# DonggeunYu/Text2Speech

Measured on AMD Instinct MI355X. Metric: WaveGlow forward audio samples/sec (batch 8x16000 per GPU), higher is better.
Workload: dtype bf16x3 (split-bf16 products, f32 accumulate); 1 GPU; WaveGlow forward, batch 8 x 16000 samples per GPU, 12 flows, n_group 8, WN 8 layers x 512 channels (reference waveglow/config.json); per_gpu_batch=8, segment_length=16000, mode=forward, parallelism=replicas, no collective

## Files before the change

text2speech_amd/csrc/conv_gemm.hip:

```cpp
#include "t2s_common.h"
#include "t2s_kernels.h"

#define B_PLANE_BYTES 16384

static __device__ __forceinline__ int swz4(int rb) {
    return (0x78 >> (rb * 2)) & 3;
}

static __device__ __forceinline__ void glds16(const void* gsrc, void* lds_dst) {
    __builtin_amdgcn_global_load_lds((const __attribute__((address_space(1))) void*)gsrc,
                                     (__attribute__((address_space(3))) void*)lds_dst, 16, 0, 0);
}

template <int EPI, int MT, bool SH = false, int NS = 2, bool X0 = false, bool RAG = false, class FMT = T2sFmt, bool A1 = false>
__global__ __launch_bounds__(512) void conv_gemm_kernel(const ConvGemmArgs a) {
    typedef typename FMT::frag8 fragT;
    constexpr int WN = 4;
    constexpr int NTH = 128 * WN;
    constexpr int NWT = 16 / WN;
    constexpr int CALL_BYTES = NTH * 16;
    constexpr int A_PLANE = MT * 64;
    constexpr int STAGE = 2 * A_PLANE + 2 * B_PLANE_BYTES;
    constexpr int MW = MT / 32;
    extern __shared__ __attribute__((aligned(16))) char smem[];
// ... 322 lines not shown
#pragma unroll
            for (int n = 0; n < NWT; ++n)
                if constexpr (!A1) acc[m][n] = FMT::mfma(al, bh[n], acc[m][n]);
#pragma unroll
            for (int n = 0; n < NWT; ++n) acc[m][n] = FMT::mfma(ah, bl[n], acc[m][n]);
#pragma unroll
            for (int n = 0; n < NWT; ++n) acc[m][n] = FMT::mfma(ah, bh[n], acc[m][n]);
            ah = ah_n;
            al = al_n;
        }
    };
    issue_a(0, 0);
    for (int u = wave; u < n_units; u += 2 * WN) issue_bunit(0, u, 0);
    asm volatile("s_waitcnt vmcnt(0)" ::: "memory");
    __syncthreads();
    const int rbase = wc * (NWT * 16) + (lane & 15);
    const int n_tap_steps = 3 * xc;
    for (int i = 0; i < n_tap_steps; ++i) {
        const int c = i / 3, tap = i - 3 * c;
        if (i + 1 < n_tap_steps) {
            const int c1 = (i + 1) / 3, tap1 = (i + 1) - 3 * c1;
            issue_a(tap1 * xc + c1, (i + 1) & 1);
        } else if (a.sc > 0) {
            issue_cond(0, (i + 1) & 1);
        }
        if (c + 1 < xc) {
            const int u = tap * (2 * WN) + wave;
            if (u < n_units) issue_bunit(c + 1, u, (c + 1) & 1);
        }
        const int row = rbase + tap * d;
        const int boff = row * 64 + (((lane >> 4) ^ swz4((row >> 2) & 3)) * 16);
        compute(Ar0 + (i & 1) * AR, Bx0 + (c & 1) * 2 * BX_PLANE, boff);
        asm volatile("s_waitcnt vmcnt(0)" ::: "memory");
        __syncthreads();
    }
    {
        const int boff0 = rbase * 64 + (((lane >> 4) ^ swz4((rbase >> 2) & 3)) * 16);
        for (int j = 0; j < a.sc; ++j) {
            const int st = (n_tap_steps + j) & 1;
            if (j + 1 < a.sc) issue_cond(j + 1, st ^ 1);
            compute(Ar0 + st * AR, Bx0 + st * 2 * BX_PLANE, boff0);
            asm volatile("s_waitcnt vmcnt(0)" ::: "memory");
            __syncthreads();
        }
    }
  }

    const int tcol = lane & 15;
    const int rq = (lane >> 4) * 4;
    if (EPI == EPI_GATE) {
        f32x4 facc[NWT];
#pragma unroll
        for (int n = 0; n < NWT; ++n) facc[n] = (f32x4){0.f, 0.f, 0.f, 0.f};
#pragma unroll
        for (int pair = 0; pair < MW / 4; ++pair) {
            u16x4 hv[2][NWT], lv[2][NWT];
#pragma unroll
            for (int half = 0; half < 2; ++half) {
                const int mp = pair * 2 + half;
                const int prow = mt * MT + wr * (MT / 2) + mp * 32 + rq;
                const f32x4 bt = *(const f32x4*)(a.bias + prow);
                const f32x4 bs = *(const f32x4*)(a.bias + prow + 16);
                const int ch = mt * (MT / 2) + wr * (MT / 4) + mp * 16 + rq;
                const bool chv = ch < a.C;
                const size_t obase = (((size_t)b * a.oc + (ch >> 5)) * a.Lp + a.halo) * 32 + (ch & 31);
#pragma unroll
                for (int n = 0; n < NWT; ++n) {
                    const int t = t0 + wc * (NWT * 16) + n * 16 + tcol;
                    u16x4 hi = {0, 0, 0, 0}, lo = {0, 0, 0, 0};
                    if (chv && t < a.L) {
                        u16x4 thi, tlo, ghi, glo;
#pragma unroll
                        for (int e = 0; e < 4; ++e) {
                            const float tv = fast_tanh(acc[2 * mp][n][e] + bt[e]);
                            const float gv = fast_sigmoid(acc[2 * mp + 1][n][e] + bs[e]);
                            u16 h, l;
                            split_fmt<FMT>(tv * gv, h, l);
                            hi[e] = h;
                            lo[e] = l;
                            split_fmt<FMT>(tv, h, l);
                            thi[e] = h;
                            tlo[e] = l;
                            split_fmt<FMT>(gv, h, l);
                            ghi[e] = h;
                            glo[e] = l;
                        }
                        const size_t o = obase + (size_t)t * 32;
                        *(u16x4*)(a.O_hi + o) = hi;
                        *(u16x4*)(a.O_lo + o) = lo;
                        if (a.T_hi) {
                            *(u16x4*)(a.T_hi + o) = thi;
                            *(u16x4*)(a.T_lo + o) = tlo;
                        }
                        if (a.G_hi) {
                            *(u16x4*)(a.G_hi + o) = ghi;
                            *(u16x4*)(a.G_lo + o) = glo;
                        }
                    }
                    hv[half][n] = hi;
                    lv[half][n] = lo;
                }
            }
            if (a.fold_A) {
                const u16* fa = a.fold_A + ((size_t)(mt * (MT / 64) + wr * (MT / 128) + pair) * 2 * 64 + lane) * 8;
                const fragT wh = *(const fragT*)fa;
                const fragT wl = *(const fragT*)(fa + 64 * 8);
#pragma unroll
                for (int n = 0; n < NWT; ++n) {
                    typedef __attribute__((ext_vector_type(8))) unsigned short u16x8;
                    const u16x8 bh8 = {hv[0][n][0], hv[0][n][1], hv[0][n][2], hv[0][n][3],
                                       hv[1][n][0], hv[1][n][1], hv[1][n][2], hv[1][n][3]};
                    const u16x8 bl8 = {lv[0][n][0], lv[0][n][1], lv[0][n][2], lv[0][n][3],
                                       lv[1][n][0], lv[1][n][1], lv[1][n][2], lv[1][n][3]};
                    const fragT bh = __builtin_bit_cast(fragT, bh8);
                    const fragT bl = __builtin_bit_cast(fragT, bl8);
                    facc[n] = FMT::mfma(wl, bh, facc[n]);
                    facc[n] = FMT::mfma(wh, bl, facc[n]);
                    facc[n] = FMT::mfma(wh, bh, facc[n]);
                }
            }
        }
        if (a.fold_A && lane < 32) {
            const int slot = mt * 2 + wr;
#pragma unroll
            for (int n = 0; n < NWT; ++n) {
                const int t = t0 + wc * (NWT * 16) + n * 16 + tcol;
                if (t >= a.L) continue;
#pragma unroll
                for (int e = 0; e < 4; ++e) {
                    float* dst = a.fold_acc + ((((size_t)slot * a.B + b) * 8 + rq + e) * a.L + t);
                    *dst = a.fold_init ? facc[n][e] : *dst + facc[n][e];
                }
            }
        }
    } else if (EPI == EPI_RESSKIP && PREX && (X0 || a.pair8)) {
      if constexpr (PREX) {
#pragma unroll
        for (int m = 0; m < MW; m += 2) {
            const int prow = mt * MT + wr * (MT / 2) + m * 16 + rq;
            const int ch = (prow & ~31) + 2 * rq;
            if (ch >= a.n_res) continue;
            const f32x4 b0 = *(const f32x4*)(a.bias + prow), b1 = *(const f32x4*)(a.bias + prow + 16);
            const size_t base = (((size_t)b * a.oc + (ch >> 5)) * a.Lp + a.halo) * 32 + (ch & 31);
#pragma unroll
            for (int n = 0; n < NWT; ++n) {
                const int t = t0 + wc * (NWT * 16) + n * 16 + tcol;
                if (t >= a.L) continue;
                u16x8_t hi, lo;
                if constexpr (RAG) {
                    if (t >= len_b) {
                        hi = lo = (u16x8_t){0, 0, 0, 0, 0, 0, 0, 0};
                        *(u16x8_t*)(a.O_hi + base + (size_t)t * 32) = hi;
                        *(u16x8_t*)(a.O_lo + base + (size_t)t * 32) = lo;
// ... 244 lines not shown
```

text2speech_amd/csrc/conv_gemm_args.h:

```cpp
#pragma once
#include "../../include/t2s_hip.h"
#include "t2s_api_common.h"
#include "t2s_kernels.h"

#include <string.h>


static inline int gate_tile_rows(int B, int C, int L) {
    const long wg256 = (long)cdiv(C, 128) * cdiv(L, 256) * B;
    return (wg256 <= 128 && C % 64 == 0) ? 128 : 256;
}
static inline int bias_act_tile_rows(int B, int Cout, int L) { return (long)cdiv(Cout, 256) * cdiv(L, 256) * B <= 64 ? 128 : 256; }
static inline int lockstep_tile_rows(int B, int C, int L) { return cdiv(C, 256) * cdiv(L, 256) * B < 200 ? 128 : 256; }
static inline int accumulate_tile_rows(int B, int Cout, int L) {
    const int wg256 = cdiv(Cout, 256) * cdiv(L, 256) * B;
    return (wg256 <= 128 || Cout % 256 == 0) && wg256 < 200 ? 128 : 256;
}
static inline bool bwd_pp256(const ConvGemmArgs& a, int rows) {
    return t2s_pp_shape_ok(a) && (long)cdiv(rows, 256) * a.n_ttiles * a.B >= 100;
}


static inline bool geometry_ok(int B, int L, int Lp, int halo, int Mpad, int rows) {
    return B > 0 && L > 0 && Lp == t2s_plane_rows(L, halo) && Mpad % 256 == 0 && Mpad >= rows;
}
static inline bool taps_ok(int taps, int dilation, int halo) {
    return taps > 0 && (taps & 1) && dilation > 0 && (taps / 2) * dilation <= halo;
}
static inline bool gate_shape_ok(int B, int C, int taps, int dilation, int L, int Lp, int halo, int Mpad) {
    return C > 0 && C % 4 == 0 && taps_ok(taps, dilation, halo) && geometry_ok(B, L, Lp, halo, Mpad, cdiv(C, 128) * 256);
}
static inline bool fold_ok(const void* fold_A, const float* fold_acc, int C) { return fold_A && fold_acc && al16(fold_A) && C % 16 == 0; }

struct ConvGemm {
    ConvGemmArgs a;

    ConvGemm(const void* A_hi, const void* A_lo, const float* bias) {
        memset(&a, 0, sizeof(a));
        a.A_hi = (const u16*)A_hi; a.A_lo = (const u16*)A_lo; a.bias = bias;
    }
    void geometry(int B, int L, int Lp, int halo, int Mpad) {
        a.B = B; a.L = L; a.Lp = Lp; a.halo = halo; a.Mpad = Mpad;
        a.n_ttiles = cdiv(L, 256);
    }
    void k_side(const void* X_hi, const void* X_lo, int xc, int taps, int dil, const void* S_hi = nullptr, const void* S_lo = nullptr,
                int sc = 0, int xbs = 0) {
        a.X_hi = (const u16*)X_hi; a.X_lo = (const u16*)X_lo; a.xc = xc; a.xbs = xbs;
        a.S_hi = (const u16*)S_hi; a.S_lo = (const u16*)S_lo; a.sc = sc;
        a.taps = taps; a.dil = dil;
        a.nk_x = taps * xc; a.nk = a.nk_x + sc;
    }
    void output(void* O_hi, void* O_lo, int oc) { a.O_hi = (u16*)O_hi; a.O_lo = (u16*)O_lo; a.oc = oc; }
    void fold(const void* fold_A, float* fold_acc, int fold_init) {
        a.fold_A = (const u16*)fold_A; a.fold_acc = fold_acc; a.fold_init = fold_init;
    }
    hipError_t launch(int epi, int rows, int mt_rows, void* stream, bool bwd_pp = false, bool h16 = false) {
        a.n_mtiles = cdiv(rows, mt_rows);
        if (h16) return t2s_launch_conv_gemm(a, epi, (hipStream_t)stream, mt_rows, true);
        if (a.ph_P > 0) return t2s_launch_gate_gemm_pp(a, (hipStream_t)stream);
        if (bwd_pp) return t2s_launch_bwd_gemm_pp(a, epi, (hipStream_t)stream);
        return t2s_launch_conv_gemm(a, epi, (hipStream_t)stream, mt_rows);
    }
};
```

text2speech_amd/csrc/gate_gemm_pp.hip:

```cpp
#include "t2s_common.h"
#include "t2s_kernels.h"

#include <stdlib.h>

#include <type_traits>

namespace {

constexpr int PP_PLANE = 16384;
constexpr int PP_HALF = 8192;
constexpr int PP_BUF = 4 * PP_PLANE;

__device__ __forceinline__ void pp_store8(u16* dst, u16x4 v) { *(u16x4*)dst = v; }

__device__ __forceinline__ int pp_swz4(int rb) { return (0x78 >> (rb * 2)) & 3; }

__device__ __forceinline__ void pp_glds16(const void* gsrc, void* lds_dst) {
    __builtin_amdgcn_global_load_lds((const __attribute__((address_space(1))) void*)gsrc,
                                     (__attribute__((address_space(3))) void*)lds_dst, 16, 0, 0);
}

struct BCursor {
    long off;
    long aoff;
// ... 276 lines not shown
    PP_STAMP(1)
    for (; ks + 2 < nk; ++ks) kstep(ks, std::true_type{});
    for (; ks < nk; ++ks) kstep(ks, std::false_type{});
    if (wr == 0) __builtin_amdgcn_s_barrier();
    PP_STAMP(2)
#undef PP_MFMA

    const int tcol = lane & 15;
    const int rq = (lane >> 4) * 4;
    int cb[4], ct[4];
    bool cok[4];
#pragma unroll
    for (int n = 0; n < 4; ++n) {
        const int col = (n >> 1) * 128 + wc * 32 + (n & 1) * 16 + tcol;
        if constexpr (PH) {
            const int bl = col / a.ph_FT, fl = col - bl * a.ph_FT;
            cb[n] = b + bl;
            ct[n] = a.ph_P * (ft * a.ph_FT + fl) + phi;
        } else {
            cb[n] = b;
            ct[n] = t0 + col;
        }
        cok[n] = cb[n] < a.B && ct[n] < a.L;
    }
  if constexpr (EPI == EPI_GATE) {
    f32x4 bt_all[4], bs_all[4];
#pragma unroll
    for (int mp = 0; mp < 4; ++mp) {
        const int prow = mt * 256 + (mp >> 1) * 128 + wr * 64 + (mp & 1) * 32 + rq;
        bt_all[mp] = *(const f32x4*)(a.bias + prow);
        bs_all[mp] = *(const f32x4*)(a.bias + prow + 16);
    }
    fragT fw_h[2] = {}, fw_l[2] = {};
    if (a.fold_A) {
#pragma unroll
        for (int pair = 0; pair < 2; ++pair) {
            const u16* fa = a.fold_A + ((size_t)(mt * 4 + pair * 2 + wr) * 2 * 64 + lane) * 8;
            fw_h[pair] = *(const fragT*)fa;
            fw_l[pair] = *(const fragT*)(fa + 64 * 8);
        }
    }
    f32x4 facc[4];
#pragma unroll
    for (int n = 0; n < 4; ++n) facc[n] = (f32x4){0.f, 0.f, 0.f, 0.f};
    if (a.fold_A && !a.fold_init && lane < 32) {
        const int slot = mt * 2 + wr;
#pragma unroll
        for (int n = 0; n < 4; ++n) {
            const int tc = cok[n] ? ct[n] : 0, bc = cok[n] ? cb[n] : 0;
#pragma unroll
            for (int e = 0; e < 4; ++e) facc[n][e] = a.fold_acc[(((size_t)slot * a.B + bc) * 8 + rq + e) * a.L + tc];
        }
    }
#pragma unroll
    for (int pair = 0; pair < 2; ++pair) {
        u16x4 hv[2][4], lv[2][4];
#pragma unroll
        for (int half = 0; half < 2; ++half) {
            const int mp = pair * 2 + half;
            constexpr float L2E = 1.4426950408889634f;
            const f32x4 bt = bt_all[mp] * (2.0f * L2E), bs = bs_all[mp] * (-L2E);
            const int ch = mt * 128 + pair * 64 + wr * 32 + half * 16 + rq;
            const bool chv = ch < a.C;
            const size_t obase = ((size_t)(ch >> 5) * a.Lp + a.halo) * 32 + (ch & 31);
#pragma unroll
            for (int n = 0; n < 4; ++n) {
                u16x4 hi = {0, 0, 0, 0}, lo = {0, 0, 0, 0};
                if (chv && cok[n]) {
                    const size_t o = obase + ((size_t)cb[n] * a.oc * a.Lp + (size_t)ct[n]) * 32;
                    if (a.G_hi) {
                        u16x4 thi, tlo, ghi, glo;
#pragma unroll
                        for (int e = 0; e < 4; ++e) {
                            const float E = __builtin_amdgcn_exp2f(fminf(fmaf(acc[2 * mp][n][e], 2.0f * L2E, bt[e]), 20.0f * L2E));
                            const float F = __builtin_amdgcn_exp2f(fmaf(acc[2 * mp + 1][n][e], -L2E, bs[e]));
                            const float tv = (E - 1.0f) * __builtin_amdgcn_rcpf(E + 1.0f);
                            const float gv = __builtin_amdgcn_rcpf(1.0f + F);
                            u16 h, l;
                            split_fmt<FMT>(tv * gv, h, l);
                            hi[e] = h;
                            lo[e] = l;
                            split_fmt<FMT>(tv, h, l);
                            thi[e] = h;
                            tlo[e] = l;
                            split_fmt<FMT>(gv, h, l);
                            ghi[e] = h;
                            glo[e] = l;
                        }
                        if (a.T_hi) {
                            pp_store8(a.T_hi + o, thi);
                            pp_store8(a.T_lo + o, tlo);
                        }
                        pp_store8(a.G_hi + o, ghi);
                        pp_store8(a.G_lo + o, glo);
                    } else {
#pragma unroll
                        for (int e = 0; e < 4; ++e) {
                            const float E = __builtin_amdgcn_exp2f(fminf(fmaf(acc[2 * mp][n][e], 2.0f * L2E, bt[e]), 20.0f * L2E));
                            const float F = __builtin_amdgcn_exp2f(fmaf(acc[2 * mp + 1][n][e], -L2E, bs[e]));
                            const float v = (E - 1.0f) * __builtin_amdgcn_rcpf((E + 1.0f) * (1.0f + F));
                            u16 h, l;
                            split_fmt<FMT>(v, h, l);
                            hi[e] = h;
                            lo[e] = l;
                        }
                    }
                    pp_store8(a.O_hi + o, hi);
                    pp_store8(a.O_lo + o, lo);
                }
                hv[half][n] = hi;
                lv[half][n] = lo;
            }
        }
        if (a.fold_A) {
            const fragT wh = fw_h[pair], wl = fw_l[pair];
#pragma unroll
            for (int n = 0; n < 4; ++n) {
                typedef __attribute__((ext_vector_type(8))) unsigned short u16x8;
                const u16x8 bh8 = {hv[0][n][0], hv[0][n][1], hv[0][n][2], hv[0][n][3],
                                   hv[1][n][0], hv[1][n][1], hv[1][n][2], hv[1][n][3]};
                const u16x8 bl8 = {lv[0][n][0], lv[0][n][1], lv[0][n][2], lv[0][n][3],
                                   lv[1][n][0], lv[1][n][1], lv[1][n][2], lv[1][n][3]};
                const fragT bh = __builtin_bit_cast(fragT, bh8);
                const fragT bl = __builtin_bit_cast(fragT, bl8);
                facc[n] = FMT::mfma(wl, bh, facc[n]);
                facc[n] = FMT::mfma(wh, bl, facc[n]);
                facc[n] = FMT::mfma(wh, bh, facc[n]);
            }
        }
    }
    if (a.fold_A && lane < 32) {
        const int slot = mt * 2 + wr;
#pragma unroll
        for (int n = 0; n < 4; ++n) {
            if (!cok[n]) continue;
#pragma unroll
            for (int e = 0; e < 4; ++e) {
                a.fold_acc[(((size_t)slot * a.B + cb[n]) * 8 + rq + e) * a.L + ct[n]] = facc[n][e];
            }
        }
    }
  } else if constexpr (EPI == EPI_RESSKIP) {
    typedef __attribute__((ext_vector_type(8))) unsigned short u16x8_t;
    if (a.pair8) {
#pragma unroll
      for (int m0 = 0; m0 < 8; m0 += 2) {
        const int grp = mt * 256 + (m0 >> 2) * 128 + wr * 64 + (m0 & 3) * 16;
        const bool rok = grp < a.n_res;
        const int chc = rok ? grp + 2 * rq : 0;
        const f32x4 b0 = *(const f32x4*)(a.bias + chc), b1 = *(const f32x4*)(a.bias + chc + 4);
        const size_t ob = ((size_t)(chc >> 5) * a.Lp + a.halo) * 32 + (chc & 31);
        u16x8_t oh[4], ol[4];
#pragma unroll
        for (int n = 0; n < 4; ++n) {
            oh[n] = (u16x8_t){0, 0, 0, 0, 0, 0, 0, 0};
            ol[n] = oh[n];
            if (rok && cok[n] && !a.res_init) {
                const size_t o = ob + ((size_t)cb[n] * a.oc * a.Lp + (size_t)ct[n]) * 32;
                oh[n] = *(const u16x8_t*)((a.R_hi ? a.R_hi : a.O_hi) + o);
                ol[n] = *(const u16x8_t*)((a.R_lo ? a.R_lo : a.O_lo) + o);
            }
        }
        if (!rok) continue;
#pragma unroll
// ... 207 lines not shown
```

text2speech_amd/csrc/t2s_api.hip:

```cpp
#include "../../include/t2s_hip.h"
#include "t2s_kernels.h"
#include "t2s_api_common.h"
#include "conv_gemm_args.h"

#include <stdlib.h>
#include <string.h>

static thread_local char g_hip_err[256] = "";

extern "C" int t2s_internal_fail_hip(int ei) {
    hipError_t e = (hipError_t)ei;
    strncpy(g_hip_err, hipGetErrorString(e), sizeof(g_hip_err) - 1);
    g_hip_err[sizeof(g_hip_err) - 1] = 0;
    return T2S_EHIP;
}


static inline bool a_operand_ok(const void* A_hi, const void* A_lo, bool h16) { return h16 ? (A_hi && al16(A_hi)) : planes_ok(A_hi, A_lo); }

static int pack_table(const t2s_pack_job* jobs, int n_jobs, long total_rows, void* stream, bool h16) {
    if (!jobs || n_jobs <= 0 || total_rows <= 0 || total_rows > 0x7fffffffL) return T2S_EINVAL;
    static_assert(sizeof(t2s_pack_job) == sizeof(PackJob), "t2s_pack_job layout");
    T2S_CHECK_HIP(t2s_launch_pack_table((const PackJob*)jobs, n_jobs, total_rows, (hipStream_t)stream, h16));
    return T2S_OK;
}

static int upsample_squeeze(const float* mel, const float* W, const float* bias, int B, int n_mel, int frames, int ksize, int stride,
                            int n_group, int L, int Lp, int halo, void* S_hi, void* S_lo, void* stream, bool h16) {
    if (!mel || !W || !bias || !S_hi || !S_lo) return T2S_EINVAL;
    if (B <= 0 || n_mel <= 0 || frames <= 0 || L <= 0 || n_group <= 0 || stride <= 0 || ksize % stride) return T2S_EINVAL;
    if (!al16(W) || !al16(S_hi) || !al16(S_lo)) return T2S_EINVAL;
    if (Lp < t2s_plane_rows(L, halo)) return T2S_EINVAL;
    if ((long)L * n_group > (long)(frames - 1) * stride + ksize) return T2S_EINVAL;
    if (n_group == 8 && (stride % 8 || ksize % 8)) return T2S_EINVAL;
    T2S_CHECK_HIP(t2s_launch_upsample_squeeze(mel, W, bias, B, n_mel, frames, ksize, stride, n_group, L, Lp, halo,
                                              (u16*)S_hi, (u16*)S_lo, (hipStream_t)stream, h16));
    return T2S_OK;
}

static int wg_start(const float* z, const float* w, const float* bias, int B, int n_group, int c_off, int n_half, int C, int L, int Lp,
                    int halo, void* X_hi, void* X_lo, void* stream, bool h16, const int* lengths = nullptr) {
    if (!z || !w || !bias || !X_hi || !X_lo) return T2S_EINVAL;
    if (B <= 0 || L <= 0 || C <= 0 || n_half <= 0 || n_half > 8 || c_off < 0 || c_off + n_half > n_group) return T2S_EINVAL;
    if (!al16(X_hi) || !al16(X_lo) || Lp < t2s_plane_rows(L, halo)) return T2S_EINVAL;
    T2S_CHECK_HIP(t2s_launch_start(z, w, bias, B, n_group, c_off, n_half, C, L, Lp, halo, (u16*)X_hi, (u16*)X_lo,
                                   (hipStream_t)stream, 0, 0, nullptr, nullptr, lengths, h16));
    return T2S_OK;
}

static int endfold_weights(const t2s_endfold_job* jobs, int n_jobs, int C, void* stream, bool h16) {
    if (!jobs || n_jobs <= 0 || C <= 0 || (size_t)8 * C * sizeof(float) > 60 * 1024) return T2S_EINVAL;
    static_assert(sizeof(t2s_endfold_job) == sizeof(EndFoldJob), "t2s_endfold_job layout");
    T2S_CHECK_HIP(t2s_launch_endfold_weights((const EndFoldJob*)jobs, n_jobs, C, (hipStream_t)stream, h16));
    return T2S_OK;
}

static int in_cond_gate_fold(const void* A_hi, const void* A_lo, const float* bias, const void* X_hi, const void* X_lo,
                             const void* S_hi, const void* S_lo, void* acts_hi, void* acts_lo, const void* fold_A, float* fold_acc,
                             int fold_init, int B, int C, int n_cond, int taps, int dilation, int L, int Lp, int halo, int Mpad,
                             void* stream, bool h16, const int* lengths = nullptr) {
    if (!a_operand_ok(A_hi, A_lo, h16) || !planes_ok(X_hi, X_lo) || !planes_ok(acts_hi, acts_lo) || !bias || !al16(bias)) return T2S_EINVAL;
    if ((n_cond > 0 && !planes_ok(S_hi, S_lo)) || !fold_ok(fold_A, fold_acc, C)) return T2S_EINVAL;
    if (!gate_shape_ok(B, C, taps, dilation, L, Lp, halo, Mpad)) return T2S_EINVAL;
    ConvGemm g(A_hi, A_lo, bias);
    g.geometry(B, L, Lp, halo, Mpad);
    g.k_side(X_hi, X_lo, cdiv(C, 32), taps, dilation, S_hi, S_lo, cdiv(n_cond, 32));
    g.output(acts_hi, acts_lo, cdiv(C, 32));
    g.fold(fold_A, fold_acc, fold_init);
    g.a.C = C;
    g.a.lengths = lengths;
    T2S_CHECK_HIP(g.launch(EPI_GATE, 2 * C, gate_tile_rows(B, C, L), stream, false, h16));
    return T2S_OK;
}

extern "C" {

int t2s_abi_version(void) { return 4; }

int t2s_sizeof_taco_decoder(void) { return (int)sizeof(t2s_taco_decoder); }
int t2s_sizeof_taco_bptt(void) { return (int)sizeof(t2s_taco_bptt); }

int t2s_operand_format(void) {
#ifdef T2S_SPLIT_F16
    return 1;
#else
    return 0;
#endif
}

const char* t2s_error_string(int code) {
    switch (code) {
        case T2S_OK: return "ok";
        case T2S_EINVAL: return "invalid argument";
        case T2S_EHIP: return "HIP runtime error";
        default: return "unknown error";
    }
}
const char* t2s_last_hip_error(void) { return g_hip_err; }

int t2s_plane_rows(int L, int halo) { return cdiv(L, 256) * 256 + 2 * halo; }
int t2s_padded_rows(int rows) { return cdiv(rows, 256) * 256; }

int t2s_pack_conv_weight(const float* v, const float* g, int g_is_scale, const float* bias_in, int O, int Cin, int Kt,
                         int perm, int C_gate, int row_off, int Mpad, int koff, int Cin_pad, void* A_hi, void* A_lo,
                         float* bias_out, int bias_accumulate, void* stream) {
    if (!v || !A_hi || !A_lo || O <= 0 || Cin <= 0 || Kt <= 0) return T2S_EINVAL;
    if (Mpad % 256 || koff % 32 || Cin_pad % 32 || Cin_pad < Cin) return T2S_EINVAL;
    if (perm == T2S_PERM_GATE) {
        if (O != 2 * C_gate || cdiv(C_gate, 128) * 256 > Mpad) return T2S_EINVAL;
    } else if (perm == T2S_PERM_NONE) {
        if (row_off < 0 || row_off + O > Mpad) return T2S_EINVAL;
    } else {
        return T2S_EINVAL;
    }
// ... 153 lines not shown
    ConvGemm g(A_hi, A_lo, bias);
    g.geometry(B, L, Lp, halo, Mpad);
    g.k_side(acts_hi, acts_lo, cdiv(C, 32), 1, 1);
    g.output(X_hi, X_lo, cdiv(C, 32));
    g.a.skip = skip; g.a.C = C; g.a.n_res = n_res; g.a.skip_init = skip_init;
    T2S_CHECK_HIP(g.launch(EPI_RESSKIP, n_res + C, 256, stream));
    return T2S_OK;
}

int t2s_wg_endfold_weights(const t2s_endfold_job* jobs, int n_jobs, int C, void* stream) {
    return endfold_weights(jobs, n_jobs, C, stream, false);
}
int t2s_wg_endfold_weights_h16(const t2s_endfold_job* jobs, int n_jobs, int C, void* stream) {
    return endfold_weights(jobs, n_jobs, C, stream, true);
}

int t2s_wg_gate_tile_rows(int B, int C, int L) {
    if (B <= 0 || C <= 0 || L <= 0) return T2S_EINVAL;
    return gate_tile_rows(B, C, L);
}

int t2s_wg_gate_fold_slots(int B, int C, int L) {
    if (B <= 0 || C <= 0 || L <= 0) return T2S_EINVAL;
    return gate_tile_rows(B, C, L) == 128 ? 2 * cdiv(C, 64) : 2 * cdiv(C, 128);
}

int t2s_wg_in_cond_gate_fold(const void* A_hi, const void* A_lo, const float* bias, const void* X_hi, const void* X_lo,
                             const void* S_hi, const void* S_lo, void* acts_hi, void* acts_lo, const void* fold_A,
                             float* fold_acc, int fold_init, int B, int C, int n_cond, int taps, int dilation, int L,
                             int Lp, int halo, int Mpad, void* stream) {
    return in_cond_gate_fold(A_hi, A_lo, bias, X_hi, X_lo, S_hi, S_lo, acts_hi, acts_lo, fold_A, fold_acc, fold_init, B, C, n_cond, taps,
                             dilation, L, Lp, halo, Mpad, stream, false);
}
int t2s_wg_in_cond_gate_fold_h16(const void* A_hi, const void* A_lo, const float* bias, const void* X_hi, const void* X_lo,
                                 const void* S_hi, const void* S_lo, void* acts_hi, void* acts_lo, const void* fold_A,
                                 float* fold_acc, int fold_init, int B, int C, int n_cond, int taps, int dilation, int L,
                                 int Lp, int halo, int Mpad, void* stream) {
    return in_cond_gate_fold(A_hi, A_lo, bias, X_hi, X_lo, S_hi, S_lo, acts_hi, acts_lo, fold_A, fold_acc, fold_init, B, C, n_cond, taps,
                             dilation, L, Lp, halo, Mpad, stream, true);
}
int t2s_wg_in_cond_gate_fold_h16_ragged(const void* A_hi, const void* A_lo, const float* bias, const void* X_hi, const void* X_lo,
                                        const void* S_hi, const void* S_lo, void* acts_hi, void* acts_lo, const void* fold_A,
                                        float* fold_acc, int fold_init, int B, int C, int n_cond, int taps, int dilation, int L,
                                        int Lp, int halo, int Mpad, const int* lengths, void* stream) {
    if (!lengths) return T2S_EINVAL;
    return in_cond_gate_fold(A_hi, A_lo, bias, X_hi, X_lo, S_hi, S_lo, acts_hi, acts_lo, fold_A, fold_acc, fold_init, B, C, n_cond, taps,
                             dilation, L, Lp, halo, Mpad, stream, true, lengths);
}

int t2s_wg_in_win_gate_fold(const void* A_hi, const void* A_lo, const float* bias, const void* W_hi, const void* W_lo,
                            const void* S_hi, const void* S_lo, void* acts_hi, void* acts_lo, const void* fold_A,
                            float* fold_acc, int fold_init, int B, int C, int n_cond, int win_chunks, int L, int Lp, int halo,
                            int Mpad, void* stream) {
    if (!planes_ok(A_hi, A_lo) || !planes_ok(W_hi, W_lo) || !planes_ok(S_hi, S_lo) || !planes_ok(acts_hi, acts_lo) || !bias ||
        !al16(bias))
        return T2S_EINVAL;
    if (!fold_ok(fold_A, fold_acc, C) || C <= 0 || n_cond <= 0 || halo < 0 || (win_chunks != 2 && win_chunks != 4)) return T2S_EINVAL;
    if (!geometry_ok(B, L, Lp, halo, Mpad, cdiv(C, 128) * 256)) return T2S_EINVAL;
    ConvGemm g(A_hi, A_lo, bias);
    g.geometry(B, L, Lp, halo, Mpad);
    g.k_side(W_hi, W_lo, win_chunks, 1, 1, S_hi, S_lo, cdiv(n_cond, 32));
    g.output(acts_hi, acts_lo, cdiv(C, 32));
    g.fold(fold_A, fold_acc, fold_init);
    g.a.C = C;
    T2S_CHECK_HIP(g.launch(EPI_GATE, 2 * C, gate_tile_rows(B, C, L), stream));
    return T2S_OK;
}

int t2s_wg_upsample_basis(const float* W, const float* bias, int n_mel, int ksize, int stride, int n_group, int Lp, int halo,
                          void* U_hi, void* U_lo, void* stream) {
    if (!W || !bias || !planes_ok(U_hi, U_lo)) return T2S_EINVAL;
    if (n_mel <= 0 || n_group <= 0 || stride <= 0 || ksize <= 0 || ksize % stride || stride % n_group) return T2S_EINVAL;
    const int ncols = (stride / n_group) * (ksize / stride) * n_mel + 1;
    if (halo < 0 || Lp != t2s_plane_rows(ncols, halo)) return T2S_EINVAL;
    T2S_CHECK_HIP(t2s_launch_upbasis_planes(W, bias, n_mel, ksize, stride, n_group, Lp, halo, (u16*)U_hi, (u16*)U_lo,
                                            (hipStream_t)stream));
    return T2S_OK;
}

int t2s_wg_compose_cond(const float* tmp, const float* bias_in, int rows, int Mpad, int P, int K2, long ld, void* A2_hi,
                        void* A2_lo, float* bias_out, void* stream) {
    if (!tmp || !bias_in || !bias_out || !planes_ok(A2_hi, A2_lo)) return T2S_EINVAL;
    if (rows <= 0 || Mpad % 256 || rows > Mpad || P <= 0 || K2 <= 0 || K2 % 32 || ld < (long)P * K2 + 1) return T2S_EINVAL;
    T2S_CHECK_HIP(t2s_launch_compose_pack(tmp, bias_in, rows, Mpad, P, K2, (int)ld, (u16*)A2_hi, (u16*)A2_lo, bias_out,
                                          (hipStream_t)stream));
    return T2S_OK;
}

int t2s_wg_melwin_planes(const float* mel, int B, int n_mel, int frames, int nlag, int Fp, void* M_hi, void* M_lo, void* stream) {
    if (!mel || !planes_ok(M_hi, M_lo)) return T2S_EINVAL;
    if (B <= 0 || n_mel <= 0 || frames <= 0 || nlag <= 0 || Fp < frames) return T2S_EINVAL;
    T2S_CHECK_HIP(t2s_launch_melwin_planes(mel, B, n_mel, frames, nlag, Fp, (u16*)M_hi, (u16*)M_lo, (hipStream_t)stream));
    return T2S_OK;
}

int t2s_wg_in_melwin_gate_fold(const void* A_hi, const void* A_lo, const void* A2_hi, const void* A2_lo, const float* bias,
                               const void* X_hi, const void* X_lo, const void* M_hi, const void* M_lo, void* acts_hi,
                               void* acts_lo, const void* fold_A, float* fold_acc, int fold_init, int B, int C, int K2,
                               int taps, int dilation, int L, int Lp, int halo, int Mpad, int P, int Fp, void* stream) {
    if (!planes_ok(A_hi, A_lo) || !planes_ok(A2_hi, A2_lo) || !planes_ok(X_hi, X_lo) || !planes_ok(M_hi, M_lo) ||
        !planes_ok(acts_hi, acts_lo) || !bias || !al16(bias))
        return T2S_EINVAL;
    if (!fold_ok(fold_A, fold_acc, C) || !gate_shape_ok(B, C, taps, dilation, L, Lp, halo, Mpad)) return T2S_EINVAL;
    if (K2 <= 0 || K2 % 32 || P <= 0) return T2S_EINVAL;
    const int F = cdiv(L, P);
    if (Fp < F || gate_tile_rows(B, C, L) != 256) return T2S_EINVAL;
    ConvGemm g(A_hi, A_lo, bias);
    g.geometry(B, L, Lp, halo, Mpad);
    g.k_side(X_hi, X_lo, cdiv(C, 32), taps, dilation, M_hi, M_lo, K2 / 32);
    g.output(acts_hi, acts_lo, cdiv(C, 32));
    g.fold(fold_A, fold_acc, fold_init);
    g.a.A2_hi = (const u16*)A2_hi; g.a.A2_lo = (const u16*)A2_lo;
    g.a.C = C;
    g.a.n_ttiles = 0;
    g.a.ph_P = P; g.a.ph_Fp = Fp;
    g.a.ph_FT = F <= 64 ? 64 : (F <= 128 ? 128 : 256);
    g.a.ph_bper = 256 / g.a.ph_FT;
    g.a.ph_nft = cdiv(F, g.a.ph_FT);
    T2S_CHECK_HIP(g.launch(EPI_GATE, 2 * C, 256, stream));
    return T2S_OK;
}

static int res_only(const void* A_hi, const void* A_lo, const float* bias, const void* acts_hi, const void* acts_lo,
                    void* X_hi, void* X_lo, int B, int C, int L, int Lp, int halo, int Mpad, int pair8, const int* lengths,
                    void* stream, bool h16 = false) {
    if (!a_operand_ok(A_hi, A_lo, h16) || !planes_ok(acts_hi, acts_lo) || !planes_ok(X_hi, X_lo) || !bias || !al16(bias)) return T2S_EINVAL;
    if (C <= 0 || C % 4 || (pair8 && C % 32) || !geometry_ok(B, L, Lp, halo, Mpad, C)) return T2S_EINVAL;
    ConvGemm g(A_hi, A_lo, bias);
    g.geometry(B, L, Lp, halo, Mpad);
    g.k_side(acts_hi, acts_lo, cdiv(C, 32), 1, 1);
    g.output(X_hi, X_lo, cdiv(C, 32));
    g.a.C = 0; g.a.n_res = C; g.a.pair8 = pair8 ? 1 : 0;
    g.a.lengths = lengths;
    T2S_CHECK_HIP(g.launch(EPI_RESSKIP, C, 128, stream, false, h16));
    return T2S_OK;
}

int t2s_wg_res_only_h16(const void* A_hi, const void* A_lo, const float* bias, const void* acts_hi, const void* acts_lo,
                        void* X_hi, void* X_lo, int B, int C, int L, int Lp, int halo, int Mpad, int pair8, void* stream) {
    return res_only(A_hi, A_lo, bias, acts_hi, acts_lo, X_hi, X_lo, B, C, L, Lp, halo, Mpad, pair8, nullptr, stream, true);
}

int t2s_wg_res_only(const void* A_hi, const void* A_lo, const float* bias, const void* acts_hi, const void* acts_lo,
                    void* X_hi, void* X_lo, int B, int C, int L, int Lp, int halo, int Mpad, int pair8, void* stream) {
    return res_only(A_hi, A_lo, bias, acts_hi, acts_lo, X_hi, X_lo, B, C, L, Lp, halo, Mpad, pair8, nullptr, stream);
}

int t2s_wg_res_only_ragged(const void* A_hi, const void* A_lo, const float* bias, const void* acts_hi, const void* acts_lo,
                           void* X_hi, void* X_lo, int B, int C, int L, int Lp, int halo, int Mpad, int pair8, const int* lengths,
                           void* stream) {
    if (!lengths) return T2S_EINVAL;
    return res_only(A_hi, A_lo, bias, acts_hi, acts_lo, X_hi, X_lo, B, C, L, Lp, halo, Mpad, pair8, lengths, stream);
}

// ... 121 lines not shown
```

text2speech_amd/csrc/t2s_kernels.h:

```cpp
#pragma once
#include <hip/hip_runtime.h>
#include <stdint.h>

typedef unsigned short u16;

enum { EPI_GATE = 0, EPI_RESSKIP = 1, EPI_BIAS_ACT = 2, EPI_GATE_BWD = 3 };
enum { ACT_NONE = 0, ACT_RELU = 1, ACT_TANH = 2 };
enum { PERM_NONE = 0, PERM_GATE = 1, PERM_PAIR8 = 2 };

struct ConvGemmArgs {
    const u16* A_hi;
    const u16* A_lo;
    const u16* X_hi;
    const u16* X_lo;
    const u16* S_hi;
    const u16* S_lo;
    const float* bias;
    u16* O_hi;
    u16* O_lo;
    float* skip;
    float* out_f32;
    int nk;
    int nk_x;
    int xc, sc, oc;
    int xbs;
    int taps, dil;
    int Mpad, Lp, halo, L, B;
    int n_mtiles, n_ttiles;
    int C;
    int n_res;
    int skip_init;
    int act;
    int f32_cl;
    u16* T_hi;
    u16* T_lo;
    u16* G_hi;
    u16* G_lo;
    int tc;
    int pair8;
    int res_init;
    const u16* R_hi;
    const u16* R_lo;
    long a_bstride;
    int ksplit;
    int k0, kchunk, kend;
    int kflat;
    const u16* fold_A;
    float* fold_acc;
    int fold_init;
    const u16* A2_hi;
    const u16* A2_lo;
    int ph_P;
    int ph_FT;
    int ph_bper;
    int ph_nft;
    int ph_Fp;
    const float* x0_z;
    const float* x0_w;
    const float* x0_b;
    int x0_G, x0_coff, x0_nh;
    const int* lengths;
};

#define T2S_RAG_SKIP_COLS 256
#ifdef __HIPCC__
static __device__ __forceinline__ void t2s_rag_zero_fold(const ConvGemmArgs& a, int mt, int b, int t0, int tid) {
    if (!a.fold_A || !a.fold_init) return;
    const int ncols = min(T2S_RAG_SKIP_COLS, a.L - t0);
    for (int idx = tid; idx < 16 * T2S_RAG_SKIP_COLS; idx += 512) {
        const int col = idx % T2S_RAG_SKIP_COLS, sj = idx / T2S_RAG_SKIP_COLS;
        if (col < ncols) a.fold_acc[(((size_t)(mt * 2 + (sj >> 3)) * a.B + b) * 8 + (sj & 7)) * a.L + t0 + col] = 0.f;
    }
}
#endif

hipError_t t2s_launch_conv_gemm(const ConvGemmArgs& a, int epi, hipStream_t stream, int mt_rows = 256, bool h16 = false);
hipError_t t2s_launch_gate_gemm_pp(const ConvGemmArgs& a, hipStream_t stream, bool h16 = false);
hipError_t t2s_launch_bwd_gemm_pp(const ConvGemmArgs& a, int epi, hipStream_t stream);
bool t2s_pp_shape_ok(const ConvGemmArgs& a);

struct WgradChunk {
    const u16* hi;
    const u16* lo;
    long bstride;
};
struct WgradClArgs {
    const WgradChunk* a_chunks;
    const WgradChunk* b_chunks;
    float* P;
    int M, N, ldp, n_mtiles, n_ntiles;
    int B, k0, k1;
    int nslab, kchunk;
    int bias_cols;
};
hipError_t t2s_launch_wgrad_cl(const WgradClArgs& a, hipStream_t stream);

struct PackArgs {
    const float* v;
    const float* g;
    const float* bias_in;
    u16* A_hi;
    u16* A_lo;
    float* bias_out;
    int O, Cin, Kt;
    int perm, C_gate;
    int Mpad;
    int koff;
    int Cin_pad;
    int bias_accumulate;
    int row_off;
    int g_is_scale;
};
hipError_t t2s_launch_pack(const PackArgs& a, hipStream_t stream);
struct PackJob {
    const float* v; const float* g; const float* bias_in; const float* bias_in2;
    u16* A_hi; u16* A_lo; float* bias_out;
    long row_start;
    long O, Cin, Kt, perm, C_gate, Mpad, koff, Cin_pad, row_off, g_is_scale;
    float* scale_out;
};
hipError_t t2s_launch_pack_table(const PackJob* jobs, int n_jobs, long total_rows, hipStream_t stream, bool h16 = false);
hipError_t t2s_launch_weightnorm_small(const float* v, const float* g, int O, int K, float* w, hipStream_t stream);

hipError_t t2s_launch_upbasis_planes(const float* W, const float* bias, int n_mel, int ksize, int stride, int n_group, int Lp,
                                     int halo, u16* U_hi, u16* U_lo, hipStream_t stream);
hipError_t t2s_launch_compose_pack(const float* tmp, const float* bias_in, int rows, int Mpad, int P, int K2, int ld, u16* A2_hi,
// ... 57 lines not shown
```

text2speech_amd/glow.py:

```python
import ctypes
import os
from collections import namedtuple

import torch
import torch.nn.functional as F

from . import _lib, sampling


class _WaveGlowLossFn(torch.autograd.Function):

    @staticmethod
    def forward(ctx, sigma, n_flows, z, *rest):
        log_s = [t.detach().to(torch.float32).contiguous() for t in rest[:n_flows]]
        dets = [t.detach() for t in rest[n_flows:]]
        d0 = dets[0]
        if all(t.dtype == torch.float32 and t.dim() == 0 and t.untyped_storage().data_ptr() == d0.untyped_storage().data_ptr()
               and t.storage_offset() == d0.storage_offset() + k for k, t in enumerate(dets)):
            log_det = d0.as_strided((n_flows,), (1,))
        else:
            log_det = torch.stack([t.to(torch.float32).reshape(()) for t in dets])
        zc = z.detach().to(torch.float32).contiguous()
        dev = zc.device
        d_z = torch.empty_like(zc) if z.requires_grad else None
# ... 507 lines not shown
        _lib.call(name, _lib.ptr(mel32), _lib.ptr(W), _lib.ptr(bias), B, up.in_channels,
                  mel32.size(2), up.kernel_size[0], up.stride[0], m.n_group, L, w["Lp"], g["halo"],
                  _lib.ptr(w["Sh"]), _lib.ptr(w["Sl"]), _lib.current_stream())
        self._keep += [mel32, W, bias]

    def _boundary(self, plan, k, z_in, z_out, B, L, w, prev=None, W=None):
        m, g = self.m, self.geom()
        c_off, n_rem, n_half = self._flow_geom(k)
        fold_acc = bes = b_end = log_s = None
        nslots = c_off_p = nh_p = 0
        if prev is not None:
            kp, log_s = prev
            c_off_p, _, nh_p = self._flow_geom(kp)
            fold_acc, nslots = w["fold_acc"], w["fold_acc"].size(0)
            bes = plan.pk["flows"][kp]["bes"]
            b_end = _f32c(m.WN[kp].end.bias)
            self._keep.append(b_end)
        name, lengths = plan.entry["boundary"]
        _lib.call(name, _lib.ptr(z_in), _lib.ptr(z_out), _lib.ptr(fold_acc), nslots, _lib.ptr(bes), g["nl"],
                  _lib.ptr(b_end), _lib.ptr(log_s), c_off_p, nh_p, _lib.ptr(W), c_off, n_rem, n_half, B, m.n_group, L, w["Lp"],
                  g["halo"], g["ks"], g["nwc"], _lib.ptr(w["Wh"]), _lib.ptr(w["Wl"]), *lengths, _lib.current_stream())

    def _wn(self, plan, k, z, B, L, w, c_off, n_half):
        m, g = self.m, self.geom()
        C, nl, ks = g["C"], g["nl"], g["ks"]
        path, P = plan.path, _lib.ptr
        fl = plan.pk["flows"][k]
        st = _lib.current_stream()
        b_start = _f32c(m.WN[k].start.bias)
        self._keep.append(b_start)
        X, S, win, acts = ((P(w[n + "h"]), P(w[n + "l"])) for n in "XSWA")
        if not path.boundary:
            name, lengths = plan.entry["start_window" if path.start_fold else "start"]
            window = ()
            if name in _START_TAKES_WINDOW:
                window = (ks, g["nwc"], *win) if path.start_fold else (0, 0, None, None)
            _lib.call(name, P(z), P(fl["w_start"]), P(b_start), B, m.n_group, c_off, n_half, C, L, w["Lp"], g["halo"], *X,
                      *window, *lengths, st)
        gate, gate_lengths = plan.entry["gate" if plan.melwin is None else "gate_melwin"]
        gate_window = plan.entry["gate_window"][0]
        res, res_lengths = plan.entry["res"]
        res_start, res_start_lengths = plan.entry["res_start"]
        pair8 = 1 if plan.pk["res_pair8"] else 0
        dims1 = (L, w["Lp"], g["halo"], g["Mpad1"])
        for i in range(nl):
            ly = fl["layers"][i]
            full_k = not (path.start_fold and i == 0)
            timed = full_k and self.gemm_events is not None and self._gemm_launch_no % self.gemm_event_stride == 0
            if full_k:
                self._gemm_launch_no += 1
            if timed:
                e0, e1 = torch.cuda.Event(enable_timing=True), torch.cuda.Event(enable_timing=True)
                e0.record()
            out = (*acts, P(ly["fold_A"]), P(w["fold_acc"]))
            if not full_k:
                _lib.call(gate_window, P(fl["A0h"]), P(fl["A0l"]), P(ly["b1"]), *win, *S, *out, 1, B, C, g["n_cond"], g["nwc"], *dims1, st)
            elif plan.melwin is not None:
                Mh, Ml, Fp, n_phase, K2 = plan.melwin
                _lib.call(gate, P(ly["A1h"]), P(ly["A1l"]), P(ly["Ach"]), P(ly["Acl"]), P(ly["b1c"]), *X, P(Mh), P(Ml), *out,
                          1 if i == 0 else 0, B, C, K2, ks, 2 ** i, *dims1, n_phase, Fp, st)
            else:
                _lib.call(gate, P(ly["A1h"]), P(ly["A1l"]), P(ly["b1"]), *X, *S, *out,
                          1 if i == 0 else 0, B, C, g["n_cond"], ks, 2 ** i, *dims1, *gate_lengths, st)
            if timed:
                e1.record()
                self.gemm_events.append((e0, e1))
            if i == nl - 1:
                continue
            weights = (P(ly["A2h"]), P(ly["A2l"]), P(ly["b2"]), *acts)
            dims2 = (B, C, L, w["Lp"], g["halo"], ly["Mpad2"])
            if path.boundary and i == 0:
                _lib.call(res_start, *weights, P(z), P(fl["w_start"]), P(b_start), m.n_group, c_off, n_half, *X, *dims2,
                          *res_start_lengths, st)
            else:
                _lib.call(res, *weights, *X, *dims2, pair8, *res_lengths, st)

    def wn_forward(self, k, audio, spect):
        self._check_inputs(audio, spect)
        dev = audio.device
        self._enter(dev)
        B, n_in, L = audio.shape
        c_off, n_rem, n_half = self._flow_geom(k)
        g = self.geom()
        if n_in != n_half or spect.size(1) != g["n_cond"] or spect.size(2) != L:
            raise ValueError("WN[%d] takes audio [B, %d, L] and spect [B, %d, L]" % (k, n_half, g["n_cond"]))
        plan = self._plan()
        self._keep = []
        plan = self._pack(plan, dev)
        w = self.workspace(B, L, dev)
        st = _lib.current_stream()
        spect32 = _f32c(spect)
        _lib.call("t2s_f32_to_planes", _lib.ptr(spect32), B, g["n_cond"], L, w["Lp"], g["halo"], _lib.ptr(w["Sh"]), _lib.ptr(w["Sl"]), st)
        z = torch.zeros(B, self.m.n_group, L, dtype=torch.float32, device=dev)
        z[:, c_off:c_off + n_half] = audio.detach().to(torch.float32)
        if plan.path.boundary:
            self._boundary(plan, k, z, None, B, L, w)
        self._wn(plan, k, z, B, L, w, c_off, n_half)
        wn_out =torch.empty(B, 2 * n_half, L, dtype=torch.float32, device=dev)
        self._end_fold(k, z, None, w["fold_acc"], wn_out, B, L, c_off, n_half, reverse=False, plan=plan)
        self._keep += [spect32, z]
        return wn_out.to(audio.dtype)

    def _end_fold(self, k, z, log_s, fold_acc, wn_out, B, L, c_off, n_half, reverse, plan=None):
        b_end = _f32c(self.m.WN[k].end.bias)
        self._keep.append(b_end)
        pk = self.packed if plan is None else plan.pk
        _lib.call("t2s_wg_end_fold_affine", _lib.ptr(fold_acc), fold_acc.size(0), _lib.ptr(pk["flows"][k]["bes"]),
# ... 412 lines not shown
```

Before: 8.166 million audio samples/s.

## Widen gate epilogue stores via permlane16 swap and skip dead last-layer acts

The gate GEMM epilogue now pairs the two 16-channel halves of each lane and shuffles them with permlane16_swap, so every lane issues one 16-byte store per plane where it previously issued two 8-byte stores, whenever C is a multiple of 16. Separately, the last WN layer of each flow no longer writes its gated activations, since only the folded skip/end path consumes them. The API validation now accepts null activation planes. The aim is less store traffic and fewer store instructions, at the cost of extra cross-lane permute instructions and more live registers in the epilogue.

Measured after the change: 8.211 million audio samples/s, median of 6. About the same (+0.5%).

```diff
diff --git a/text2speech_amd/csrc/conv_gemm.hip b/text2speech_amd/csrc/conv_gemm.hip
--- a/text2speech_amd/csrc/conv_gemm.hip
+++ b/text2speech_amd/csrc/conv_gemm.hip
@@ -398,53 +398,93 @@
         f32x4 facc[NWT];
 #pragma unroll
         for (int n = 0; n < NWT; ++n) facc[n] = (f32x4){0.f, 0.f, 0.f, 0.f};
+        const bool st_acts = a.O_hi != nullptr;
+        const bool st16 = (a.C & 15) == 0;
+        const int pc = t2s_gate_piece16_ch(lane);
 #pragma unroll
         for (int pair = 0; pair < MW / 4; ++pair) {
             u16x4 hv[2][NWT], lv[2][NWT];
+            f32x4 bt2[2], bs2[2];
 #pragma unroll
             for (int half = 0; half < 2; ++half) {
-                const int mp = pair * 2 + half;
-                const int prow = mt * MT + wr * (MT / 2) + mp * 32 + rq;
-                const f32x4 bt = *(const f32x4*)(a.bias + prow);
-                const f32x4 bs = *(const f32x4*)(a.bias + prow + 16);
-                const int ch = mt * (MT / 2) + wr * (MT / 4) + mp * 16 + rq;
-                const bool chv = ch < a.C;
-                const size_t obase = (((size_t)b * a.oc + (ch >> 5)) * a.Lp + a.halo) * 32 + (ch & 31);
-#pragma unroll
-                for (int n = 0; n < NWT; ++n) {
-                    const int t = t0 + wc * (NWT * 16) + n * 16 + tcol;
-                    u16x4 hi = {0, 0, 0, 0}, lo = {0, 0, 0, 0};
+                const int prow = mt * MT + wr * (MT / 2) + (pair * 2 + half) * 32 + rq;
+                bt2[half] = *(const f32x4*)(a.bias + prow);
+                bs2[half] = *(const f32x4*)(a.bias + prow + 16);
+            }
+            const int ch0 = mt * (MT / 2) + wr * (MT / 4) + pair * 32;
+            const size_t cbase = (((size_t)b * a.oc + (ch0 >> 5)) * a.Lp + a.halo) * 32;
+            const bool pv = ch0 + pc < a.C;
+#pragma unroll
+            for (int n = 0; n < NWT; ++n) {
+                const int t = t0 + wc * (NWT * 16) + n * 16 + tcol;
+                const size_t ocol = cbase + (size_t)t * 32;
+                u16x4 hi[2], lo[2], thi[2], tlo[2], ghi[2], glo[2];
+#pragma unroll
+                for (int half = 0; half < 2; ++half) {
+                    const int mp = pair * 2 + half;
+                    const f32x4 bt = bt2[half], bs = bs2[half];
+                    const int ch = ch0 + half * 16 + rq;
+                    const bool chv = ch < a.C;
+                    hi[half] = lo[half] = thi[half] = tlo[half] = ghi[half] = glo[half] = (u16x4){0, 0, 0, 0};
                     if (chv && t < a.L) {
-                        u16x4 thi, tlo, ghi, glo;
 #pragma unroll
                         for (int e = 0; e < 4; ++e) {
                             const float tv = fast_tanh(acc[2 * mp][n][e] + bt[e]);
                             const float gv = fast_sigmoid(acc[2 * mp + 1][n][e] + bs[e]);
                             u16 h, l;
                             split_fmt<FMT>(tv * gv, h, l);
-                            hi[e] = h;
-                            lo[e] = l;
+                            hi[half][e] = h;
+                            lo[half][e] = l;
                             split_fmt<FMT>(tv, h, l);
-                            thi[e] = h;
-                            tlo[e] = l;
+                            thi[half][e] = h;
+                            tlo[half][e] = l;
                             split_fmt<FMT>(gv, h, l);
-                            ghi[e] = h;
-                            glo[e] = l;
+                            ghi[half][e] = h;
+                            glo[half][e] = l;
                         }
-                        const size_t o = obase + (size_t)t * 32;
-                        *(u16x4*)(a.O_hi + o) = hi;
-                        *(u16x4*)(a.O_lo + o) = lo;
-                        if (a.T_hi) {
-                            *(u16x4*)(a.T_hi + o) = thi;
-                            *(u16x4*)(a.T_lo + o) = tlo;
+                        if (!st16) {
+                            const size_t o = ocol + (half * 16 + rq);
+                            if (st_acts) {
+                                *(u16x4*)(a.O_hi + o) = hi[half];
+                                *(u16x4*)(a.O_lo + o) = lo[half];
+                            }
+                            if (a.T_hi) {
+                                *(u16x4*)(a.T_hi + o) = thi[half];
+                                *(u16x4*)(a.T_lo + o) = tlo[half];
+                            }
+                            if (a.G_hi) {
+                                *(u16x4*)(a.G_hi + o) = ghi[half];
+                                *(u16x4*)(a.G_lo + o) = glo[half];
+                            }
                         }
-                        if (a.G_hi) {
-                            *(u16x4*)(a.G_hi + o) = ghi;
-                            *(u16x4*)(a.G_lo + o) = glo;
+                    }
+                    hv[half][n] = hi[half];
+                    lv[half][n] = lo[half];
+                }
+                if (st16) {
+                    const bool ok = pv && t < a.L;
+                    const size_t o = ocol + pc;
+                    if (st_acts) {
+                        const t2s_u32x4 h16 = t2s_gate_piece16(hi[0], hi[1]), l16 = t2s_gate_piece16(lo[0], lo[1]);
+                        if (ok) {
+                            t2s_store16(a.O_hi + o, h16);
+                            t2s_store16(a.O_lo + o, l16);
                         }
                     }
-                    hv[half][n] = hi;
-                    lv[half][n] = lo;
+                    if (a.T_hi) {
+                        const t2s_u32x4 th16 = t2s_gate_piece16(thi[0], thi[1]), tl16 = t2s_gate_piece16(tlo[0], tlo[1]);
+                        if (ok) {
+                            t2s_store16(a.T_hi + o, th16);
+                            t2s_store16(a.T_lo + o, tl16);
+                        }
+                    }
+                    if (a.G_hi) {
+                        const t2s_u32x4 gh16 = t2s_gate_piece16(ghi[0], ghi[1]), gl16 = t2s_gate_piece16(glo[0], glo[1]);
+                        if (ok) {
+                            t2s_store16(a.G_hi + o, gh16);
+                            t2s_store16(a.G_lo + o, gl16);
+                        }
+                    }
                 }
             }
             if (a.fold_A) {
diff --git a/text2speech_amd/csrc/conv_gemm_args.h b/text2speech_amd/csrc/conv_gemm_args.h
--- a/text2speech_amd/csrc/conv_gemm_args.h
+++ b/text2speech_amd/csrc/conv_gemm_args.h
@@ -30,6 +30,7 @@
 static inline bool gate_shape_ok(int B, int C, int taps, int dilation, int L, int Lp, int halo, int Mpad) {
     return C > 0 && C % 4 == 0 && taps_ok(taps, dilation, halo) && geometry_ok(B, L, Lp, halo, Mpad, cdiv(C, 128) * 256);
 }
+static inline bool acts_ok(const void* acts_hi, const void* acts_lo) { return (!acts_hi && !acts_lo) || planes_ok(acts_hi, acts_lo); }
 static inline bool fold_ok(const void* fold_A, const float* fold_acc, int C) { return fold_A && fold_acc && al16(fold_A) && C % 16 == 0; }
 
 struct ConvGemm {
diff --git a/text2speech_amd/csrc/gate_gemm_pp.hip b/text2speech_amd/csrc/gate_gemm_pp.hip
--- a/text2speech_amd/csrc/gate_gemm_pp.hip
+++ b/text2speech_amd/csrc/gate_gemm_pp.hip
@@ -352,24 +352,29 @@
             for (int e = 0; e < 4; ++e) facc[n][e] = a.fold_acc[(((size_t)slot * a.B + bc) * 8 + rq + e) * a.L + tc];
         }
     }
+    const bool st_acts = a.O_hi != nullptr;
+    const bool st16 = (a.C & 15) == 0;
+    const int pc = t2s_gate_piece16_ch(lane);
 #pragma unroll
     for (int pair = 0; pair < 2; ++pair) {
         u16x4 hv[2][4], lv[2][4];
-#pragma unroll
-        for (int half = 0; half < 2; ++half) {
-            const int mp = pair * 2 + half;
-            constexpr float L2E = 1.4426950408889634f;
-            const f32x4 bt = bt_all[mp] * (2.0f * L2E), bs = bs_all[mp] * (-L2E);
-            const int ch = mt * 128 + pair * 64 + wr * 32 + half * 16 + rq;
-            const bool chv = ch < a.C;
-            const size_t obase = ((size_t)(ch >> 5) * a.Lp + a.halo) * 32 + (ch & 31);
-#pragma unroll
-            for (int n = 0; n < 4; ++n) {
-                u16x4 hi = {0, 0, 0, 0}, lo = {0, 0, 0, 0};
+        constexpr float L2E = 1.4426950408889634f;
+        const int ch0 = mt * 128 + pair * 64 + wr * 32;
+        const size_t cbase = ((size_t)(ch0 >> 5) * a.Lp + a.halo) * 32;
+        const bool pv = ch0 + pc < a.C;
+#pragma unroll
+        for (int n = 0; n < 4; ++n) {
+            u16x4 hi[2], lo[2], thi[2], tlo[2], ghi[2], glo[2];
+            const size_t ocol = cbase + ((size_t)cb[n] * a.oc * a.Lp + (size_t)ct[n]) * 32;
+#pragma unroll
+            for (int half = 0; half < 2; ++half) {
+                const int mp = pair * 2 + half;
+                const f32x4 bt = bt_all[mp] * (2.0f * L2E), bs = bs_all[mp] * (-L2E);
+                const int ch = ch0 + half * 16 + rq;
+                const bool chv = ch < a.C;
+                hi[half] = lo[half] = thi[half] = tlo[half] = ghi[half] = glo[half] = (u16x4){0, 0, 0, 0};
                 if (chv && cok[n]) {
-                    const size_t o = obase + ((size_t)cb[n] * a.oc * a.Lp + (size_t)ct[n]) * 32;
                     if (a.G_hi) {
-                        u16x4 thi, tlo, ghi, glo;
 #pragma unroll
                         for (int e = 0; e < 4; ++e) {
                             const float E = __builtin_amdgcn_exp2f(fminf(fmaf(acc[2 * mp][n][e], 2.0f * L2E, bt[e]), 20.0f * L2E));
@@ -378,21 +383,15 @@
                             const float gv = __builtin_amdgcn_rcpf(1.0f + F);
                             u16 h, l;
                             split_fmt<FMT>(tv * gv, h, l);
-                            hi[e] = h;
-                            lo[e] = l;
+                            hi[half][e] = h;
+                            lo[half][e] = l;
                             split_fmt<FMT>(tv, h, l);
-                            thi[e] = h;
-                            tlo[e] = l;
+                            thi[half][e] = h;
+                            tlo[half][e] = l;
                             split_fmt<FMT>(gv, h, l);
-                            ghi[e] = h;
-                            glo[e] = l;
+                            ghi[half][e] = h;
+                            glo[half][e] = l;
                         }
-                        if (a.T_hi) {
-                            pp_store8(a.T_hi + o, thi);
-                            pp_store8(a.T_lo + o, tlo);
-                        }
-                        pp_store8(a.G_hi + o, ghi);
-                        pp_store8(a.G_lo + o, glo);
                     } else {
 #pragma unroll
                         for (int e = 0; e < 4; ++e) {
@@ -401,15 +400,53 @@
                             const float v = (E - 1.0f) * __builtin_amdgcn_rcpf((E + 1.0f) * (1.0f + F));
                             u16 h, l;
                             split_fmt<FMT>(v, h, l);
-                            hi[e] = h;
-                            lo[e] = l;
+                            hi[half][e] = h;
+                            lo[half][e] = l;
                         }
                     }
-                    pp_store8(a.O_hi + o, hi);
-                    pp_store8(a.O_lo + o, lo);
+                    if (!st16) {
+                        const size_t o = ocol + (half * 16 + rq);
+                        if (a.G_hi) {
+                            if (a.T_hi) {
+                                pp_store8(a.T_hi + o, thi[half]);
+                                pp_store8(a.T_lo + o, tlo[half]);
+                            }
+                            pp_store8(a.G_hi + o, ghi[half]);
+                            pp_store8(a.G_lo + o, glo[half]);
+                        }
+                        if (st_acts) {
+                            pp_store8(a.O_hi + o, hi[half]);
+                            pp_store8(a.O_lo + o, lo[half]);
+                        }
+                    }
                 }
-                hv[half][n] = hi;
-                lv[half][n] = lo;
+                hv[half][n] = hi[half];
+                lv[half][n] = lo[half];
+            }
+            if (st16) {
+                const bool ok = pv && cok[n];
+                const size_t o = ocol + pc;
+                if (a.G_hi) {
+                    if (a.T_hi) {
+                        const t2s_u32x4 th16 = t2s_gate_piece16(thi[0], thi[1]), tl16 = t2s_gate_piece16(tlo[0], tlo[1]);
+                        if (ok) {
+                            t2s_store16(a.T_hi + o, th16);
+                            t2s_store16(a.T_lo + o, tl16);
+                        }
+                    }
+                    const t2s_u32x4 gh16 = t2s_gate_piece16(ghi[0], ghi[1]), gl16 = t2s_gate_piece16(glo[0], glo[1]);
+                    if (ok) {
+                        t2s_store16(a.G_hi + o, gh16);
+                        t2s_store16(a.G_lo + o, gl16);
+                    }
+                }
+                if (st_acts) {
+                    const t2s_u32x4 h16 = t2s_gate_piece16(hi[0], hi[1]), l16 = t2s_gate_piece16(lo[0], lo[1]);
+                    if (ok) {
+                        t2s_store16(a.O_hi + o, h16);
+                        t2s_store16(a.O_lo + o, l16);
+                    }
+                }
             }
         }
         if (a.fold_A) {
diff --git a/text2speech_amd/csrc/t2s_api.hip b/text2speech_amd/csrc/t2s_api.hip
--- a/text2speech_amd/csrc/t2s_api.hip
+++ b/text2speech_amd/csrc/t2s_api.hip
@@ -59,7 +59,7 @@
                              const void* S_hi, const void* S_lo, void* acts_hi, void* acts_lo, const void* fold_A, float* fold_acc,
                              int fold_init, int B, int C, int n_cond, int taps, int dilation, int L, int Lp, int halo, int Mpad,
                              void* stream, bool h16, const int* lengths = nullptr) {
-    if (!a_operand_ok(A_hi, A_lo, h16) || !planes_ok(X_hi, X_lo) || !planes_ok(acts_hi, acts_lo) || !bias || !al16(bias)) return T2S_EINVAL;
+    if (!a_operand_ok(A_hi, A_lo, h16) || !planes_ok(X_hi, X_lo) || !acts_ok(acts_hi, acts_lo) || !bias || !al16(bias)) return T2S_EINVAL;
     if ((n_cond > 0 && !planes_ok(S_hi, S_lo)) || !fold_ok(fold_A, fold_acc, C)) return T2S_EINVAL;
     if (!gate_shape_ok(B, C, taps, dilation, L, Lp, halo, Mpad)) return T2S_EINVAL;
     ConvGemm g(A_hi, A_lo, bias);
@@ -319,7 +319,7 @@
                             const void* S_hi, const void* S_lo, void* acts_hi, void* acts_lo, const void* fold_A,
                             float* fold_acc, int fold_init, int B, int C, int n_cond, int win_chunks, int L, int Lp, int halo,
                             int Mpad, void* stream) {
-    if (!planes_ok(A_hi, A_lo) || !planes_ok(W_hi, W_lo) || !planes_ok(S_hi, S_lo) || !planes_ok(acts_hi, acts_lo) || !bias ||
+    if (!planes_ok(A_hi, A_lo) || !planes_ok(W_hi, W_lo) || !planes_ok(S_hi, S_lo) || !acts_ok(acts_hi, acts_lo) || !bias ||
         !al16(bias))
         return T2S_EINVAL;
     if (!fold_ok(fold_A, fold_acc, C) || C <= 0 || n_cond <= 0 || halo < 0 || (win_chunks != 2 && win_chunks != 4)) return T2S_EINVAL;
@@ -366,7 +366,7 @@
                                void* acts_lo, const void* fold_A, float* fold_acc, int fold_init, int B, int C, int K2,
                                int taps, int dilation, int L, int Lp, int halo, int Mpad, int P, int Fp, void* stream) {
     if (!planes_ok(A_hi, A_lo) || !planes_ok(A2_hi, A2_lo) || !planes_ok(X_hi, X_lo) || !planes_ok(M_hi, M_lo) ||
-        !planes_ok(acts_hi, acts_lo) || !bias || !al16(bias))
+        !acts_ok(acts_hi, acts_lo) || !bias || !al16(bias))
         return T2S_EINVAL;
     if (!fold_ok(fold_A, fold_acc, C) || !gate_shape_ok(B, C, taps, dilation, L, Lp, halo, Mpad)) return T2S_EINVAL;
     if (K2 <= 0 || K2 % 32 || P <= 0) return T2S_EINVAL;
diff --git a/text2speech_amd/csrc/t2s_kernels.h b/text2speech_amd/csrc/t2s_kernels.h
--- a/text2speech_amd/csrc/t2s_kernels.h
+++ b/text2speech_amd/csrc/t2s_kernels.h
@@ -72,6 +72,23 @@
         if (col < ncols) a.fold_acc[(((size_t)(mt * 2 + (sj >> 3)) * a.B + b) * 8 + (sj & 7)) * a.L + t0 + col] = 0.f;
     }
 }
+
+typedef __attribute__((ext_vector_type(2))) unsigned int t2s_u32x2;
+typedef __attribute__((ext_vector_type(4))) unsigned int t2s_u32x4;
+template <class V8>
+static __device__ __forceinline__ t2s_u32x4 t2s_gate_piece16(V8 half0, V8 half1) {
+    static_assert(sizeof(V8) == 8, "one lane's four 16-bit values of an m-tile");
+    const t2s_u32x2 a = __builtin_bit_cast(t2s_u32x2, half0), b = __builtin_bit_cast(t2s_u32x2, half1);
+#if defined(__HIP_DEVICE_COMPILE__)
+    const t2s_u32x2 r0 = __builtin_amdgcn_permlane16_swap(a[0], b[0], false, false);
+    const t2s_u32x2 r1 = __builtin_amdgcn_permlane16_swap(a[1], b[1], false, false);
+    return (t2s_u32x4){r0[0], r1[0], r0[1], r1[1]};
+#else
+    return (t2s_u32x4){a[0], a[1], b[0], b[1]};
+#endif
+}
+static __device__ __forceinline__ int t2s_gate_piece16_ch(int lane) { return ((lane >> 4) & 1) * 16 + (lane >> 5) * 8; }
+static __device__ __forceinline__ void t2s_store16(u16* dst, t2s_u32x4 v) { *(t2s_u32x4*)dst = v; }
 #endif
 
 hipError_t t2s_launch_conv_gemm(const ConvGemmArgs& a, int epi, hipStream_t stream, int mt_rows = 256, bool h16 = false);
diff --git a/text2speech_amd/glow.py b/text2speech_amd/glow.py
--- a/text2speech_amd/glow.py
+++ b/text2speech_amd/glow.py
@@ -583,7 +583,8 @@
             if timed:
                 e0, e1 = torch.cuda.Event(enable_timing=True), torch.cuda.Event(enable_timing=True)
                 e0.record()
-            out = (*acts, P(ly["fold_A"]), P(w["fold_acc"]))
+            acts_out = (None, None) if i == nl - 1 else acts
+            out = (*acts_out, P(ly["fold_A"]), P(w["fold_acc"]))
             if not full_k:
                 _lib.call(gate_window, P(fl["A0h"]), P(fl["A0l"]), P(ly["b1"]), *win, *S, *out, 1, B, C, g["n_cond"], g["nwc"], *dims1, st)
             elif plan.melwin is not None:
```
